# blackccpie/another_raytracer

Hardware: AMD Instinct MI355X
Metric: Msamples/sec (primary+secondary rays) at 1920x1080x1024spp; 1/2/4/8 GPU (higher is better)
Workload: dtype f64

## Files before the change

### another_raytracer_amd/_lib.py

```python
import ctypes
import os

try:
    import torch
except ImportError:
    pass

_HERE = os.path.dirname(os.path.abspath(__file__))
LIB_PATH = os.environ.get("ART_LIB") or os.path.join(_HERE, "libart.so")

RT_OK = 0
RT_FP64 = 0
RT_ABI_VERSION = 5
RT_OUT_DEVICE, RT_PROFILE, RT_GLOBAL_SCENE, RT_SPLIT_SHADE, RT_ADAPTIVE, RT_WAVEFRONT, RT_PARALLEL_IMAGES = 1, 2, 4, 8, 16, 32, 64
RT_GUIDE_DOUBLES = 10
RT_DN_NO_DEMODULATE = 256
RT_Q_ANY_HIT, RT_Q_NO_MEDIA = 512, 1024
RT_HIT_DOUBLES = 12
ERRORS = {-1: "RT_E_INVALID", -2: "RT_E_SCENE", -3: "RT_E_DEVICE", -4: "RT_E_INTERNAL"}


class rt_camera(ctypes.Structure):
    _fields_ = [("lookfrom", ctypes.c_double * 3), ("lookat", ctypes.c_double * 3), ("vup", ctypes.c_double * 3),
                ("vfov", ctypes.c_double), ("aspect", ctypes.c_double), ("aperture", ctypes.c_double),
# ... 77 lines not shown
    "rt_option_set": (_I, [ctypes.c_char_p, _D]),
    "rt_option_get": (_I, [ctypes.c_char_p, _DP]),
    "rt_scene_build": (_I, [ctypes.c_char_p, ctypes.c_char_p, _I, ctypes.POINTER(_P)]),
    "rt_scene_info_get": (_I, [_P, ctypes.POINTER(rt_scene_info)]),
    "rt_scene_dump": (_S, [_P, ctypes.c_char_p, _S]),
    "rt_scene_destroy": (None, [_P]),
    "rt_scene_save": (_I, [_P, ctypes.c_char_p]),
    "rt_scene_load": (_I, [ctypes.c_char_p, _I, ctypes.POINTER(_P)]),
    "rt_render": (_I, [_P, ctypes.POINTER(rt_camera), ctypes.POINTER(rt_params), _P, _P, ctypes.POINTER(rt_stats)]),
    "rt_render_progressive": (_I, [_P, ctypes.POINTER(rt_camera), ctypes.POINTER(rt_params), _P, _P, rt_progress_fn, _P,
                                   ctypes.POINTER(rt_stats)]),
    "rt_trace_rays": (_I, [_P, _P, ctypes.c_int64, ctypes.c_int32, _P, _P]),
    "rt_query_rays": (_I, [_P, ctypes.POINTER(rt_query_params), _P, _P, ctypes.c_int64, _P, _P]),
    "rt_radiance_rays": (_I, [_P, ctypes.POINTER(rt_radiance_params), _P, _P, ctypes.c_int64, _P, ctypes.POINTER(rt_stats)]),
    "rt_camera_rays": (_I, [ctypes.POINTER(rt_camera), ctypes.POINTER(rt_params), ctypes.c_uint32, _I, _P, _P]),
    "rt_render_views": (_I, [_P, ctypes.POINTER(rt_camera), _P, ctypes.c_int32, ctypes.POINTER(rt_params), _P, _P, ctypes.POINTER(rt_stats)]),
    "rt_render_guides": (_I, [_P, ctypes.POINTER(rt_camera), ctypes.POINTER(rt_params), _P, _P]),
    "rt_denoise": (_I, [_I, ctypes.POINTER(rt_denoise_params), _P, _P, ctypes.c_int32, _P, _P, _P, _DP]),
    "rt_render_denoised": (_I, [_P, ctypes.POINTER(rt_camera), ctypes.POINTER(rt_params), ctypes.POINTER(rt_denoise_params), _P, _P,
                                ctypes.POINTER(rt_stats)]),
    "rt_render_noise_target": (_I, [_P, ctypes.POINTER(rt_camera), ctypes.POINTER(rt_params), ctypes.POINTER(rt_noise_params), _P, _P, _P, _P,
                                    ctypes.POINTER(rt_stats), ctypes.POINTER(rt_noise_result)]),
    "rt_image_load": (_I, [ctypes.c_char_p, ctypes.POINTER(ctypes.c_int32), ctypes.POINTER(ctypes.c_int32), ctypes.POINTER(ctypes.c_int32),
                           ctypes.POINTER(ctypes.POINTER(ctypes.c_uint8))]),
    "rt_image_free": (None, [ctypes.POINTER(ctypes.c_uint8)]),
    "rt_local_rows": (_I, [ctypes.POINTER(rt_params), ctypes.POINTER(ctypes.c_int32)]),
    "rt_band_block_rows": (_I, [ctypes.c_int32, ctypes.c_int32, ctypes.c_int32]),
    "rt_unpack_bands": (_I, [_P, _S, _P, _S, ctypes.c_int32, ctypes.c_int32, ctypes.c_int32, ctypes.c_int32, ctypes.c_int32, _P]),
    "rt_multi_create": (_I, [ctypes.c_char_p, ctypes.c_char_p, _IP, _I, ctypes.POINTER(_P)]),
    "rt_multi_from_graph": (_I, [_P, _IP, _I, ctypes.POINTER(_P)]),
# ... 133 lines not shown
```

### another_raytracer_amd/csrc/abi.cpp

```cpp
#include <chrono>
#include <cmath>
#include <cstdlib>
#include <cstring>
#include <exception>
#include <stdexcept>
#include <memory>
#include <new>
#include <string>
#include <vector>

#include "art.h"
#include "denoise.h"
#include "imagedec.h"
#include "multi.h"
#include "renderer.h"
#include "scenefile.h"
#include "objmesh.h"
#include "options.h"
#include "pass_plan.h"
#include "scene.h"

namespace art {
int device_count();
}
// ... 373 lines not shown
    if (view_paths > art::kMaxPassSlots)
        return fail(RT_E_INVALID, "rt_render_views: one view of width * height * spp = " + std::to_string(view_paths) + " paths exceeds kMaxPassSlots = "
                                  "2^31 paths per launch: render such frames with rt_render, which splits a frame into passes");
    if (nviews == 0) return RT_OK;
    if (!out_rgb8) return fail(RT_E_INVALID, "rt_render_views: out_rgb8 must be non-NULL");
    return guard(RT_E_DEVICE, [&] {
        std::vector<art::CameraRec> recs(static_cast<size_t>(nviews));
        for (int32_t v = 0; v < nviews; ++v) recs[static_cast<size_t>(v)] = camera_of(&cams[v]);
        art::RenderStats st;
        s->device_renderer().render_views(recs.data(), seeds, static_cast<size_t>(nviews), render_params(p), out_rgb8, out_accum, stats ? &st : nullptr);
        if (stats) {
            fill_stats(st, stats);
            stats->extend_variant = stats->kernel_lds_mode = -1;
        }
        return RT_OK;
    });
}

int rt_camera_rays(const rt_camera* cam, const rt_params* p, uint32_t sample_base, int device, double* rays_out, uint64_t* rng_out) {
    std::string why;
    if (!cam || !rays_out) return fail(RT_E_INVALID, "rt_camera_rays: camera and rays_out must be non-NULL");
    if (!p) return fail(RT_E_INVALID, "params is NULL");
    if (device < 0) return fail(RT_E_INVALID, "device must be >= 0");
    rt_params q = *p;
    q.max_depth = 0;
    if (!valid_params(&q, why)) return fail(RT_E_INVALID, why);
    if (p->flags & ~RT_OUT_DEVICE) return fail(RT_E_INVALID, "rt_camera_rays takes RT_OUT_DEVICE only");
    if (p->stream && !(p->flags & RT_OUT_DEVICE)) return fail(RT_E_INVALID, "rt_camera_rays: stream needs RT_OUT_DEVICE");
    const uint64_t rows = static_cast<uint64_t>(art::band_local_rows(p->height, p->band_rows, p->band_count, p->band_index));
    const uint64_t npix_pad = static_cast<uint64_t>((p->width + 7) / 8) * ((rows + 7) / 8) * 64u;
// ... 365 lines not shown
```

### another_raytracer_amd/csrc/device_scene.h

```cpp
#pragma once
#include <algorithm>
#include <vector>

#include "hip_check.h"
#include "path_work.h"
#include "scene.h"

namespace art {

struct DeviceScene {
    std::vector<void*> allocs;
    DevScene view{};
    bool media = false;
    uint32_t features = F_ALL;
    int max_stack = kMaxStackDepth;
    uint32_t mat_types = (1u << kNumMatTypes) - 1;
    bool tex_basic = false;
    bool lds_scene = false;
    bool lds_shade = false;
    bool codes16 = false;
    uint32_t leaf_shift = 0;
    bool tex_bary = false;
    size_t bytes = 0;

    template <class T>
    const T* upload(const std::vector<T>& v) {
        if (v.empty()) return nullptr;
        void* p = nullptr;
        HIP_OK(hipMalloc(&p, v.size() * sizeof(T)));
        HIP_OK(hipMemcpy(p, v.data(), v.size() * sizeof(T), hipMemcpyHostToDevice));
        allocs.push_back(p);
        bytes += v.size() * sizeof(T);
        return static_cast<const T*>(p);
    }
// ... 15 lines not shown
```

### another_raytracer_amd/csrc/device_scene.hip

```cpp
#include "device_scene.h"

#include <cmath>
#include <cstring>
#include <limits>
#include <unordered_map>

#include "options.h"

namespace art {

static std::vector<uint8_t> lds_scene_image(const FlatScene& f, uint32_t& nmov, bool& shade_ok) {
    std::vector<uint8_t> img;
    nmov = 0;
    shade_ok = false;
    if ((f.features & ~kFeatSpheres) != 0 || f.nodes.empty() || f.nodes.size() > kLdsNodeCap || f.primrefs.size() > kLdsSlotCap ||
        f.world.size() > kPathsWorldCap || f.objs.size() > kPathsWorldCap ||
        f.spheres.size() > kLdsRefIndexMask || std::max(extend_lds_bytes(true, stack_rows(f.max_stack)), paths_lds_bytes(stack_rows(f.max_stack))) > kLdsPerCu)
        return img;
    for (int32_t w : f.world)
        if (w < 0 || static_cast<size_t>(w) >= f.objs.size() || f.objs[w].kind != OBJ_BVH) return img;
    for (uint32_t ref : f.primrefs) {
        if (primref_type(ref) != PRIM_SPHERE) return img;
        const SphereRec& sp = f.spheres[primref_index(ref)];
        if (sp.flags & SPH_MOVING) {
            if (sp.t0 != 0.0 || sp.dt != 1.0 || sp.d[0] != 0.0 || sp.d[2] != 0.0) return img;
            ++nmov;
        }
    }
// ... 65 lines not shown
            } else if (mat.type == MAT_DIELECTRIC) {
                const double inv = 1.0 / mat.ir;
                double r0f = (1.0 - inv) / (1.0 + inv), r0b = (1.0 - mat.ir) / (1.0 + mat.ir);
                r0f = r0f * r0f;
                r0b = r0b * r0b;
                const double d3[3] = {inv, r0f, r0b};
                entry[sp.mat] = static_cast<int32_t>(put_entry(d3, mat.ir));
            } else {
                shade_ok = false;
            }
        }
        const uint16_t mi = static_cast<uint16_t>(entry[sp.mat] < 0 ? 0 : entry[sp.mat]);
        put(kLdsOffMatIdx + sl * 2, &mi, 2);
    }
    if (nent > kLdsMatCap) shade_ok = false;
    return img;
}


static std::vector<uint32_t> pair_align_leaves(const std::vector<uint32_t>& primrefs, std::vector<BvhNode>& nodes,
                                               std::vector<ObjRec>& objs, std::vector<uint8_t>& pad) {
    std::vector<std::pair<uint32_t, uint32_t>> leaves;
    for (const BvhNode& b : nodes)
        for (int c = 0; c < 4; ++c)
            if (b.child[c] < 0 && b.child[c] != kNodeEmpty) leaves.emplace_back(leaf_first(b.child[c]), leaf_count(b.child[c]));
    for (const auto& o : objs)
        if (o.kind == OBJ_BVH && o.b != kNodeEmpty) leaves.emplace_back(leaf_first(o.b), leaf_count(o.b));
    std::sort(leaves.begin(), leaves.end());
    leaves.erase(std::unique(leaves.begin(), leaves.end()), leaves.end());
    std::unordered_map<uint32_t, uint32_t> moved;
// ... 161 lines not shown
    }
    ds.view.world = ds.upload(f.world);
    ds.view.mats = ds.upload(mats);
    ds.view.texs = ds.upload(f.texs);
    ds.view.perlins = ds.upload(f.perlins);
    {
        std::vector<uint8_t> ib(kUvTableBytes + sizeof(ImageRec) * f.images.size(), 0);
        std::memcpy(ib.data(), glibc_trig_data::kTrigHost, sizeof(glibc_trig_data::kTrigHost));
        if (!f.images.empty()) std::memcpy(ib.data() + kUvTableBytes, f.images.data(), sizeof(ImageRec) * f.images.size());
        ds.view.images = reinterpret_cast<const ImageRec*>(ds.upload(ib) + kUvTableBytes);
    }
    ds.view.texels = ds.upload(f.texels);
    {
        uint32_t nmov = 0;
        bool shade_ok = false;
        const std::vector<uint8_t> img = ds.leaf_shift ? std::vector<uint8_t>() : lds_scene_image(f, nmov, shade_ok);
        if (!img.empty()) {
            ds.view.lds_image = ds.upload(img);
            ds.lds_scene = true;
            ds.lds_shade = shade_ok;
        }
    }
    ds.view.n_nodes = static_cast<uint32_t>(f.nodes.size());
    ds.view.n_objs = static_cast<uint32_t>(f.objs.size());
    ds.view.n_mats = static_cast<uint32_t>(f.mats.size());
    ds.view.n_primrefs = static_cast<uint32_t>(f.primrefs.size());
    ds.view.n_tris = static_cast<uint32_t>(f.tris.size());
    ds.view.nworld = static_cast<int32_t>(f.world.size());
    for (int a = 0; a < 3; ++a) ds.view.bg[a] = f.background[a];
    ds.media = f.has_media;
    ds.features = f.features;
// ... 25 lines not shown
```

### another_raytracer_amd/csrc/k_paths.hip

```cpp
#include "launch.h"
#include "path_pool.h"
#include "path_work.h"

namespace art {

struct __align__(16) PoolRay {
    double2 a, b, c;
    double2 d, e;
    uint64_t rng;
    uint32_t slot, depth;
};
static_assert(sizeof(PoolRay) == 96, "pool entries are six 16-B pieces");
struct PathPool {
    PoolRay* base;
    uint32_t count;
    uint32_t cur, end;
    bool exhausted;
    __device__ __forceinline__ void init(void* pool, uint32_t block, uint32_t nblocks, uint32_t waves_per_block, uint32_t w) {
        const uint32_t per_xcd = (nblocks + kXcds - 1) / kXcds;
        const uint32_t wave = ((block % kXcds) * per_xcd + block / kXcds) * waves_per_block + w;
        base = static_cast<PoolRay*>(pool) + static_cast<size_t>(wave) * kPoolCap;
        count = cur = end = 0;
        exhausted = false;
    }
    __device__ __forceinline__ bool batch(const PassGeom& sg, const CameraRec& sc, uint32_t* next_slot, uint32_t lane, PathState& st,
                                          uint32_t& q) {
        if (cur == end) {
            const uint32_t chunk = sg.chunk;
            uint32_t nb = 0;
            if (lane == 0) nb = atomicAdd(next_slot, chunk);
            nb = __builtin_amdgcn_readfirstlane(nb);
            cur = nb;
            end = nb + chunk;
        }
        const uint32_t b = cur;
        cur += 64;
        q = b + lane;
        __asm__ volatile("" ::: "memory");
        if (b + 64u >= sg.P) exhausted = true;
        int lx, ly;
        uint32_t qi, j;
        slot_split(sg, q, qi, j);
        if (!(q < sg.P && slot_pixel(sg, qi, lx, ly))) return false;
        cam_ray(sg, sc, j, lx, ly, st.ray, st.rng);
        st.T = mk(1.0, 1.0, 1.0);
        return true;
    }
    __device__ __forceinline__ void push(uint64_t m, uint32_t rank, bool busy, const PathState& st, uint32_t q, int depth) {
        if (busy) {
            PoolRay& e = base[pool_push_pos(count, rank)];
            e.a = make_double2(st.ray.o.x, st.ray.o.y);
            e.b = make_double2(st.ray.o.z, st.ray.d.x);
            e.c = make_double2(st.ray.d.y, st.ray.d.z);
            e.d = make_double2(st.ray.tm, st.T.x);
            e.e = make_double2(st.T.y, st.T.z);
            e.rng = st.rng;
            e.slot = q;
// ... 2 lines not shown
        count += static_cast<uint32_t>(__popcll(m));
        __asm__ volatile("" ::: "memory");
    }
    __device__ __forceinline__ void pop(uint32_t rank, PathState& st, uint32_t& q, int& depth) const {
        const PoolRay& e = base[pool_pop_pos(count, rank)];
        const double2 a = e.a, b = e.b, c = e.c, d = e.d, f = e.e;
        st.ray.o = mk(a.x, a.y, b.x);
        st.ray.d = mk(b.y, c.x, c.y);
        st.ray.tm = d.x;
        st.T = mk(d.y, f.x, f.y);
        st.rng = e.rng;
        q = e.slot;
        depth = static_cast<int>(e.depth);
    }
};
__global__ __launch_bounds__(kBlockL, 1) void k_paths(DevScene S0, PassGeom g, CameraRec cam, Work w, uint32_t* next_slot) {
    constexpr int B = kBlockL;
    extern __shared__ __align__(16) uint8_t smem[];
    const uint8_t* lds = smem;
    StackT<true>* stk = reinterpret_cast<StackT<true>*>(smem + kLdsImageBytes) + B + stack_column<true>(threadIdx.x);
    JumpEntry* jt = reinterpret_cast<JumpEntry*>(smem + kLdsImageBytes + paths_stack_bytes(g.stack));
    CameraRec& s_cam = *reinterpret_cast<CameraRec*>(smem + kLdsImageBytes + paths_stack_bytes(g.stack) + kJumpBytes);
    PassGeom& s_g = *reinterpret_cast<PassGeom*>(smem + kLdsImageBytes + paths_stack_bytes(g.stack) + kJumpBytes + sizeof(CameraRec));
    stk[-B] = static_cast<StackT<true>>(kNodeEmpty);
    load_lds_image<B>(S0.lds_image, smem);
    if (threadIdx.x < static_cast<uint32_t>(kJumpEntries)) jt[threadIdx.x] = pcg_jump(3u * threadIdx.x);
    if (threadIdx.x == 0) {
        s_cam = cam;
        s_g = g;
        if (g.list_mode) {
// ... 12 lines not shown
        S.world = reinterpret_cast<const int32_t*>(wb);
        S.objs = reinterpret_cast<const ObjRec*>(ob);
    }
    __syncthreads();
    const uint32_t lane = __lane_id();
    const uint64_t below = (1ull << lane) - 1ull;
    const V3 bg = mk(S.bg[0], S.bg[1], S.bg[2]);
    bool busy = false;
    uint32_t q = 0;
    int depth = 0;
    PathState st;
    unsigned long long segs = 0;
#ifdef ART_STATS
    unsigned long long tm_load = 0, tm_trace = 0, tm_shade = 0, tm_app = 0, tm_fb = 0, tm_prev = __builtin_amdgcn_s_memtime();
#endif
    PathPool pp;
    pp.init(w.pool, blockIdx.x, gridDim.x, B / 64, threadIdx.x / 64);
    for (;;) {
        const uint64_t m_busy = __ballot(busy);
        const uint32_t n_idle = 64u - static_cast<uint32_t>(__popcll(m_busy));
        const bool fb = pool_batch_due(pp.exhausted, pp.count, n_idle);
        bool act;
        if (fb) {
#ifdef ART_STATS
            if (lane == 0) atomicAdd(&g_art_stats[51], static_cast<unsigned long long>(__popcll(m_busy)));
#endif
            if (m_busy) pp.push(m_busy, static_cast<uint32_t>(__popcll(m_busy & below)), busy, st, q, depth);
            act = pp.batch(s_g, s_cam, next_slot, lane, st, q);
            depth = 0;
        } else {
            const uint32_t npop = pool_pop_count(pp.count, n_idle);
            if (npop) {
                const uint32_t rank = static_cast<uint32_t>(__popcll(~m_busy & below));
                if (!busy && rank < npop) {
                    pp.pop(rank, st, q, depth);
                    busy = true;
                }
                pp.count -= npop;
            } else if (m_busy == 0) {
                ART_TICK(tm_load);
                break;
            }
            act = busy;
        }
        ART_TICK((fb ? tm_fb : tm_load));
        double t = 0.0;
        HitOut h{0, 0, kMatUnknown};
        bool hitw = false;
        if (act) {
            ++segs;
            hitw = trace_world<kFeatSpheres, B, true>(S, lds, st.ray, stk, st.rng, t, h);
#if ART_LDS_LEAF_NOREF
            if (hitw) h.mt = reinterpret_cast<const uint32_t*>(lds + kLdsOffRef)[h.obj >> 16] >> kLdsRefMatShift;
#endif
        }
        __asm__ volatile("s_waitcnt vmcnt(0)" ::: "memory");
        ART_TICK((fb ? tm_fb : tm_trace));
        const bool need = act && hitw && (h.mt == MAT_LAMBERTIAN || h.mt == MAT_METAL) && depth + 1 < g.max_depth;
        const V3 ps = coop_unit_sphere(need, st.rng, jt);
        bool cont = false;
        if (act) {
            st.L = mk(0.0, 0.0, 0.0);
            if (hitw) {
                cont = shade_hit_lds(lds, h.obj >> 16, h.mt, t, depth + 1 >= g.max_depth, st, &ps);
            } else {
                st.L = st.L + st.T * bg;
// ... 46 lines not shown
```

### another_raytracer_amd/csrc/kernels_unity.hip

```cpp
#include "kernels.hip"
#include "k_paths.hip"
#include "k_paths_g_mesh.hip"
#include "radiance_rays.hip"
#include "device_scene.hip"
#include "renderer.hip"
```

### another_raytracer_amd/csrc/launch.h

```cpp
#pragma once
#include <functional>

#include "device_scene.h"
#include "path_work.h"

namespace art {

enum ExtendVariant { EXT_GLOBAL = 0, EXT_LDS = 1, EXT_FUSED = 2, EXT_MEGA = 3, EXT_MEGA_G = 4 };
int extend_variant(const DeviceScene& ds, int flags);
struct KernelId {
    uint32_t f = 0, tf = 0;
    int lm = -1;
};

bool static_lds_is_zero(const void* kernel);
int blocks_per_cu(const void* kernel, int block, size_t lds);
KernelId launch_paths_g(uint32_t feat, bool tex_basic, bool tex_bary, bool codes16, uint32_t leaf_shift, int num_cu, hipStream_t st,
                        const DevScene& S, const PassGeom& g, const CameraRec& cam, const Work& w, uint32_t* next_slot);
void bounce(const DeviceScene& ds, int variant, int num_cu, hipStream_t st, const PassGeom& g, const CameraRec& cam,
            const Work& w, int d, const std::function<void()>& mark);
void launch_accum(hipStream_t st, const PassGeom& g, const Work& w, double* qsum, uint32_t m);
void launch_finalize(hipStream_t st, const double* acc, uint8_t* rgb, uint32_t n, int spp);
void launch_adapt_corners(hipStream_t st, uint32_t* list, int W, int sqx, uint32_t nsq);
void launch_adapt_store(hipStream_t st, const uint32_t* list, uint32_t n, const double* acc, int spp, int32_t* work);
// ... 33 lines not shown
    ResRec* res;
    uint32_t* next;
    unsigned long long* segments;
    uint32_t P, spp, chunk;
    uint32_t npix;
    uint32_t stack;
    int32_t max_depth;
    int32_t W, H;
    double inv_w1, inv_h1;
    FastDiv fd_spp, fd_npix, fd_w;
};
void launch_radiance_views(const DeviceScene& ds, int flags, int num_cu, hipStream_t st, const ViewsJob& job, uint32_t npixels, const double background[3]);
void launch_camera_rays(hipStream_t st, const PassGeom& g, const CameraRec& cam, double* rays, uint64_t* rng);
void launch_paths(int num_cu, hipStream_t st, const DevScene& S, const PassGeom& g, const CameraRec& cam, const Work& w,
                  uint32_t* next_slot);
size_t pool_bytes(int variant, int num_cu);

}
```

### another_raytracer_amd/csrc/options.cpp

```cpp
#include "options.h"

#include <algorithm>
#include <atomic>
#include <cmath>
#include <cstdlib>
#include <cstring>
#include <limits>

namespace art {

namespace {

struct OptDef {
    const char* name;
    double def, lo, hi;
    bool integer;
};
constexpr double kInf = std::numeric_limits<double>::infinity();
const OptDef kDefs[static_cast<int>(Opt::kCount)] = {
    {"compile.world_merge", 2, 0, 2, true},
    {"compile.hoist", 1, 0, 1, true},
    {"bvh.collapse", 0, 0, 1, true},
    {"bvh.collapse_ci", 0.6, 0, 1e6, false},
    {"bvh.dp_binary_leaf", 1, 1, 16, true},
    {"bvh.sah_ci", 1.5, 0, 1e6, false},
    {"bvh.sah_leaf", 4, 1, 16, true},
    {"bvh.sbvh", 1.5, 0, 1e6, false},
    {"bvh.sbvh_alpha", 1e-5, 0, 1e6, false},
    {"render.codes16", 1, 0, 1, true},
    {"render.lds_nodes_max", 4294967295.0, 0, 4294967295.0, true},
    {"render.leaf2", 1, 0, 1, true},
    {"render.tex_bary", 1, 0, 1, true},
    {"denoise.lds_iterations", 2, 0, 2, true},
    {"query.any_sorted", 0, 0, 1, true},
    {"views.max_paths", 0, 0, 2147483648.0, true},
    {"multi.timeout_ms", std::numeric_limits<double>::quiet_NaN(), 0, kInf, false},
    {"multi.rccl_blocking", 0, 0, 1, true},
    {"test.fault_workspace_bytes", 0, 0, 1.8e19, true},
    {"test.fault_gather_abort", 0, 0, 1, true},
    {"test.fault_rccl_group", 0, 0, 2, true},
};

std::atomic<double> g_val[static_cast<int>(Opt::kCount)];
std::atomic<bool> g_init{false};

void init_once() {
    if (g_init.load(std::memory_order_acquire)) return;
    static const bool done = [] {
        opt_reset_all();
        g_init.store(true, std::memory_order_release);
// ... 54 lines not shown
```

### another_raytracer_amd/csrc/options.h

```cpp
#pragma once
#include <cstddef>

namespace art {

enum class Opt : int {
    WorldMerge,
    Hoist,
    BvhCollapse,
    CollapseCi,
    DpBinaryLeaf,
    SahCi,
    SahLeaf,
    Sbvh,
    SbvhAlpha,
    Codes16,
    LdsNodesMax,
    Leaf2,
    TexBary,
    DenoiseLdsIterations,
    QueryAnySorted,
    ViewsMaxPaths,
    MultiTimeoutMs,
    RcclBlocking,
    FaultWorkspaceBytes,
    FaultGatherAbort,
    FaultRcclGroup,
    kCount
};

double opt(Opt o);
bool opt_set(const char* name, double value, const char** why);
bool opt_get(const char* name, double* value);
void opt_reset_all();

}
```

### another_raytracer_amd/csrc/path_work.h

```cpp
#pragma once
#include <hip/hip_runtime.h>

#include <cstdint>

#include "device.h"
#include "pass_plan.h"

namespace art {

struct PathRec {
    double2 a, b, c, e;
    double2 f, g, h, i;
};
static_assert(sizeof(PathRec) == 128, "PathRec is two 64-B lines");
struct PathState {
    Ray ray;
    V3 T, L;
    uint64_t rng;
};
__device__ __forceinline__ void load_path(const PathRec* P, uint32_t q, PathState& s, bool full) {
    const PathRec& p = P[q];
    const double2 a = p.a, b = p.b, c = p.c, e = p.e;
    s.ray.o = mk(a.x, a.y, b.x);
    s.ray.d = mk(b.y, c.x, c.y);
// ... 79 lines not shown
    uint32_t nlist;
    uint32_t chunk;
    uint32_t lds_ring;
    uint32_t list_mode;
};
struct Work {
    PathRec* paths;
    HitRecD* hits;
    ResRec* res;
    uint32_t* active[2];
    uint32_t* mq;
    uint32_t* counters;
    unsigned long long* segments;
    double* acc;
    void* pool;
};
__host__ __device__ __forceinline__ uint32_t* counter(const Work& w, int d, int kind, int s) {
    return w.counters + (static_cast<size_t>((d * kQueueKinds + kind) * kShards + s)) * kCounterStride;
}

__device__ __forceinline__ int global_row(const PassGeom& g, int ly) {
    const uint32_t b = g.fd_band_rows.div(static_cast<uint32_t>(ly));
    return static_cast<int>(b) * (g.band_rows * g.band_count) + g.band_index * g.band_rows + (ly - static_cast<int>(b) * g.band_rows);
}
__device__ __forceinline__ void slot_split(const PassGeom& g, uint32_t slot, uint32_t& qi, uint32_t& j) {
    const uint32_t a = g.fd_npix.div(slot), b = slot - a * g.npix_pad;
    qi = g.list_mode ? a : b;
    j = g.list_mode ? b : a;
}
__device__ __forceinline__ bool slot_pixel(const PassGeom& g, uint32_t qi, int& lx, int& ly) {
// ... 268 lines not shown
```

### another_raytracer_amd/csrc/renderer.h

```cpp
#pragma once
#include <cstdint>
#include <functional>

#include "art.h"
#include "layout.h"
#include "noise_target.h"
#include "scene.h"

namespace art {

struct RenderParams {
    int width = 0, height = 0, spp = 1, max_depth = 50;
    uint64_t seed = 0;
    int fp_mode = RT_FP64;
    int band_rows = 1, band_count = 1, band_index = 0;
    int samples_per_pass = 0;
    int flags = 0;
    void* stream = nullptr;
    double background[3] = {0, 0, 0};
    std::function<bool(int samples_done)> on_pass;
};

struct RenderStats {
    uint64_t segments = 0, primary = 0;
// ... 21 lines not shown
    ~Renderer();
    Renderer(const Renderer&) = delete;
    Renderer& operator=(const Renderer&) = delete;
    void upload();
    void render(const CameraRec& cam, const RenderParams& p, uint8_t* out_rgb, double* out_acc, RenderStats& stats);
    void trace_rays(const double* rays, size_t n, bool global_scene, double* t_out, double* n_out);
    void query_rays(const double* rays, const double* t_max, size_t n, bool device, bool global_scene, bool any_hit, bool no_media, void* stream,
                    double* hits, uint8_t* occluded);
    void radiance_rays(const RadianceParams& p, const double* rays, const uint64_t* rng, size_t n, double* radiance, RenderStats* stats);
    void render_views(const CameraRec* cams, const uint64_t* seeds, size_t nviews, const RenderParams& p, uint8_t* out_rgb, double* out_acc,
                      RenderStats* stats);
    static void camera_rays(int device, const CameraRec& cam, const RenderParams& p, uint32_t sample_base, double* rays_out, uint64_t* rng_out);
    void render_guides(const CameraRec& cam, const RenderParams& p, double* guides, double* rays_out);
    void render_noise_target(const CameraRec& cam, const RenderParams& p, const NoiseParams& np, uint8_t* out_rgb, double* out_acc,
                             int32_t* out_count, double* out_moments, RenderStats& stats, NoiseResult& result);
    int device() const;
    size_t scene_bytes() const;
    const FlatScene& flat() const;

private:
    Impl* impl_;
};

}
```

### another_raytracer_amd/csrc/renderer.hip

```cpp
#include "renderer.h"

#include <algorithm>
#include <cstdio>
#include <cstdlib>
#include <cstring>
#include <vector>

#include "launch.h"
#include "options.h"
#include "pass_plan.h"
#include "view_plan.h"
#include "workspace.h"

namespace art {

struct Renderer::Impl {
    int device = 0;
    int num_cu = 256;
    hipStream_t own_stream = nullptr;
    FlatScene flat;
    DeviceScene s64;
    bool up64 = false;
    DeviceBuffer ws{true};
    hipEvent_t ev[2] = {nullptr, nullptr};
    std::vector<ViewRec> view_table;
// ... 35 lines not shown
    g.band_index = p.band_index;
    g.tiles_x = static_cast<uint32_t>((p.width + 7) / 8);
    const uint32_t tiles_y = static_cast<uint32_t>((nrows + 7) / 8);
    g.npix_pad = g.tiles_x * tiles_y * 64u;
    g.max_depth = p.max_depth;
    g.seed = p.seed;
    g.seed_mix = splitmix64(p.seed);
    g.fd_tiles_x = FastDiv::make(g.tiles_x);
    g.fd_band_rows = FastDiv::make(static_cast<uint32_t>(p.band_rows));
    g.fd_w = FastDiv::make(static_cast<uint32_t>(p.width));
    g.fd_npix = FastDiv::make(g.npix_pad);
    g.inv_w1 = 1.0 / static_cast<double>(p.width - 1);
    g.inv_h1 = 1.0 / static_cast<double>(p.height - 1);
    g.stack = stack;
    return g;
}
static size_t counter_words(int max_depth) { return static_cast<size_t>(std::max(max_depth + 1, 4)) * kQueueKinds * kShards * kCounterStride; }

struct ProfileMarks {
    std::vector<hipEvent_t> ev;
    size_t used = 0;
    ~ProfileMarks() { for (auto e : ev) if (e) (void)hipEventDestroy(e); }
    void reserve(size_t n) {
        while (ev.size() < n) {
            ev.push_back(nullptr);
            HIP_OK(hipEventCreate(&ev.back()));
        }
    }
    void mark(hipStream_t stream) {
        reserve(used + 1);
// ... 258 lines not shown
    launch_adapt_fill(f.stream, b.ad_work, f.drgb, p.width, f.nrows, b.sqx, b.ad_f0, b.ad_f1, b.ad_f2);
    return traced * static_cast<uint64_t>(b.spp_t);
}

void Renderer::render(const CameraRec& cam, const RenderParams& p, uint8_t* out_rgb, double* out_acc, RenderStats& stats) {
    if (p.fp_mode != RT_FP64) throw std::runtime_error("fp_mode must be RT_FP64");
    upload();
    Impl& I = *impl_;
    Frame f{I, I.s64, cam, p};
    const bool images = (p.flags & RT_PARALLEL_IMAGES) != 0, adaptive = (p.flags & RT_ADAPTIVE) != 0;
    RenderBufs b{};
    b.spp_t = images ? 4 * (p.spp / 4) : p.spp, b.out_rgb = out_rgb, b.out_acc = out_acc;
#ifdef ART_TRACE
    trace_setup();
#endif
    if (!begin_frame(f, stats, b.spp_t, true, adaptive ? 4 : 1, [&](Carver& c) {
        const bool wf = !f.mega;
        f.w.paths = c.take<PathRec>(f.Pmax, wf);
        f.w.hits = c.take<HitRecD>(f.Pmax, wf);
        f.w.res = c.take<ResRec>(f.Pmax);
        f.w.active[0] = c.take<uint32_t>(static_cast<size_t>(kShards) * f.g.cap, wf);
        f.w.active[1] = c.take<uint32_t>(static_cast<size_t>(kShards) * f.g.cap, wf);
        f.w.mq = c.take<uint32_t>(static_cast<size_t>(kMatSegs) * f.g.cap, wf);
        f.w.counters = c.take<uint32_t>(counter_words(p.max_depth));
        f.w.segments = c.take<unsigned long long>(1);
        f.w.acc = c.take<double>(3 * f.local_pix);
        f.drgb = c.take<uint8_t>(3 * f.local_pix);
        double* qsum = c.take<double>(3 * f.local_pix, images);
        b.qsum = images ? qsum : nullptr;
        f.w.pool = c.take<char>(pool_bytes(f.variant, I.num_cu));
        b.ad_work = c.take<int32_t>(3 * f.local_pix, adaptive);
        b.ad_lists = c.take<uint32_t>(f.local_pix + 4 * 64, adaptive);
        b.ad_f0 = c.take<uint8_t>(21 * (f.local_pix / (kBig * kBig)), adaptive);
        b.ad_count = c.take<uint32_t>(1, adaptive);
    })) return;
    b.ad_f1 = b.ad_f0 + f.local_pix / (kBig * kBig), b.ad_f2 = b.ad_f1 + 4 * (f.local_pix / (kBig * kBig));
    b.sqx = p.width / kBig, b.nsq = static_cast<uint32_t>(b.sqx) * static_cast<uint32_t>(f.nrows / kBig);
    uint32_t ad_counts[4] = {0, 0, 0, 0};
    uint64_t primary = 0;
    if (!adaptive) primary = render_whole(f, b);
    else if (f.mega && f.k == static_cast<uint32_t>(b.spp_t) && !images && !p.on_pass) adaptive_device_counted(f, b, ad_counts);
    else primary = adaptive_host_counted(f, b);
    end_frame(f, stats, out_rgb, adaptive ? nullptr : out_acc);
    stats.primary = primary + (static_cast<uint64_t>(ad_counts[0]) + ad_counts[1] + ad_counts[2] + ad_counts[3]) * static_cast<uint64_t>(b.spp_t);
}

void Renderer::upload() {
    HIP_OK(hipSetDevice(impl_->device));
    if (!impl_->up64) {
        build_device_scene(impl_->flat, impl_->s64);
        impl_->up64 = true;
    }
}

void Renderer::trace_rays(const double* rays, size_t n, bool global_scene, double* t_out, double* n_out) {
    upload();
    const DeviceScene& ds = impl_->s64;
    if (n == 0) return;
    if (n > (1u << 30)) throw std::runtime_error("too many rays");
// ... 330 lines not shown
```

### another_raytracer_amd/engine.py

```python
import ctypes
import enum

import numpy as np

from ._lib import RT_ADAPTIVE, RT_DN_NO_DEMODULATE, RT_FP64, RT_GUIDE_DOUBLES, rt_denoise_params, RT_PARALLEL_IMAGES, rt_progress_fn, RT_GLOBAL_SCENE, RT_OUT_DEVICE, RT_PROFILE, RT_SPLIT_SHADE, RT_WAVEFRONT, check, dvec, lib, rt_camera, rt_params, rt_stats
from .scene import compile_world


class tracer_constants:
    aspect_ratio = 4.0 / 3.0
    image_width = 720
    image_height = int(image_width / aspect_ratio)
    color_channels = 3
    samples_per_pixel = 100
    max_depth = 50


class engine_mode(enum.Enum):
    single = 0
    adaptive = 1
    parallel_stripes = 2
    parallel_images = 3


# ... 135 lines not shown
        rows = check(lib.rt_local_rows(ctypes.byref(p), None), "rt_local_rows")
        nbytes = rows * self.width * 3
        ptr, dev = _pointer(output_image, nbytes)
        acc_ptr = None
        if accum is not None:
            acc_ptr, acc_dev = _pointer(accum.view(np.uint8) if isinstance(accum, np.ndarray) else accum, nbytes * 8)
            if acc_dev != dev:
                raise ValueError("output_image and accum must both live on the host or both on the device")
        if dev:
            p.flags |= RT_OUT_DEVICE
        st = rt_stats()
        check(lib.rt_render(self._scene, ctypes.byref(self.cam.c), ctypes.byref(p), ctypes.c_void_p(ptr),
                            ctypes.c_void_p(acc_ptr) if acc_ptr else None, ctypes.byref(st)), "engine.run")
        self.stats = st.as_dict()
        return int(round(st.ms))

    def render_guides(self, guides=None, rays=None, band_rows=None, band_count=1, band_index=0, stream=None):
        if self._scene is None:
            raise ValueError("no scene set")
        p = self.params(band_rows, band_count, band_index, RT_GLOBAL_SCENE if self.global_scene else 0, stream)
        rows = check(lib.rt_local_rows(ctypes.byref(p), None), "rt_local_rows")
        n = rows * self.width
        if guides is None:
            guides = np.empty((rows, self.width, RT_GUIDE_DOUBLES), np.float64)
        ptr, dev = _f64_pointer(guides, RT_GUIDE_DOUBLES * n, "guides")
        rays_ptr = None
        if rays is not None:
            rays_ptr, rays_dev = _f64_pointer(rays, 7 * n, "rays")
            if rays_dev != dev:
                raise ValueError("guides and rays must both live on the host or both on the device")
# ... 126 lines not shown
```

### include/art.h

```cpp
#ifndef ART_H
#define ART_H

#include <stddef.h>
#include <stdint.h>

#ifdef __cplusplus
extern "C" {
#endif

#define RT_ABI_VERSION 5

#define RT_OK 0
#define RT_E_INVALID (-1)
#define RT_E_SCENE (-2)
#define RT_E_DEVICE (-3)
#define RT_E_INTERNAL (-4)

#define RT_FP64 0
#define RT_OUT_DEVICE 1
#define RT_PROFILE 2
#define RT_GLOBAL_SCENE 4
#define RT_SPLIT_SHADE 8
#define RT_ADAPTIVE 16
#define RT_WAVEFRONT 32
// ... 79 lines not shown
int rt_query_rays(rt_scene* scene, const rt_query_params* q, const double* rays, const double* t_max, int64_t n, double* hits,
                  uint8_t* occluded);
typedef struct rt_radiance_params {
    int32_t flags;
    int32_t spp;
    int32_t max_depth;
    uint32_t sample_base;
    uint64_t seed;
    uint64_t id_base;
    void* stream;
    double background[3];
} rt_radiance_params;
int rt_radiance_rays(rt_scene* scene, const rt_radiance_params* q, const double* rays, const uint64_t* rng, int64_t n, double* radiance,
                     rt_stats* stats);
int rt_camera_rays(const rt_camera* cam, const rt_params* params, uint32_t sample_base, int device, double* rays_out, uint64_t* rng_out);
int rt_render_views(rt_scene* scene, const rt_camera* cams, const uint64_t* seeds, int32_t nviews, const rt_params* params, uint8_t* out_rgb8,
                    double* out_accum, rt_stats* stats);
int rt_local_rows(const rt_params* params, int32_t* rows_out);
int rt_band_block_rows(int32_t height, int32_t band_rows, int32_t n);
int rt_unpack_bands(const uint8_t* packed, size_t packed_bytes, uint8_t* frame, size_t frame_bytes, int32_t width, int32_t height,
                    int32_t band_rows, int32_t n, int32_t flags, void* stream);

#define RT_GUIDE_DOUBLES 10
int rt_render_guides(rt_scene* scene, const rt_camera* cam, const rt_params* params, double* guides, double* rays_out);
#define RT_DN_NO_DEMODULATE 256
typedef struct rt_denoise_params {
    int32_t width, height;
    int32_t iterations;
    int32_t normal_squarings;
    double sigma_color;
// ... 84 lines not shown
```

Baseline: 20430.

## Cull primary rays per 8x8 tile with precomputed sphere candidate lists

Adds a pre-pass kernel that builds, for each 8x8 pixel tile, a depth-sorted list of up to 15 spheres whose conservative cone bound, padded for lens and motion blur, can reach the tile. In the megakernel, first-bounce rays intersect only that short list from LDS instead of walking the full BVH, and tiles that overflow fall back to the normal traversal. It is on by default for LDS-resident sphere scenes at 72 spp or more, and adds an extra launch plus a debug API. Correctness depends on the conservative bound staying valid.

```diff
diff --git a/another_raytracer_amd/_lib.py b/another_raytracer_amd/_lib.py
--- a/another_raytracer_amd/_lib.py
+++ b/another_raytracer_amd/_lib.py
@@ -115,6 +115,7 @@
     "rt_query_rays": (_I, [_P, ctypes.POINTER(rt_query_params), _P, _P, ctypes.c_int64, _P, _P]),
     "rt_radiance_rays": (_I, [_P, ctypes.POINTER(rt_radiance_params), _P, _P, ctypes.c_int64, _P, ctypes.POINTER(rt_stats)]),
     "rt_camera_rays": (_I, [ctypes.POINTER(rt_camera), ctypes.POINTER(rt_params), ctypes.c_uint32, _I, _P, _P]),
+    "rt_tile_candidates": (_I, [_P, ctypes.POINTER(rt_camera), ctypes.POINTER(rt_params), _P, ctypes.c_int64]),
     "rt_render_views": (_I, [_P, ctypes.POINTER(rt_camera), _P, ctypes.c_int32, ctypes.POINTER(rt_params), _P, _P, ctypes.POINTER(rt_stats)]),
     "rt_render_guides": (_I, [_P, ctypes.POINTER(rt_camera), ctypes.POINTER(rt_params), _P, _P]),
     "rt_denoise": (_I, [_I, ctypes.POINTER(rt_denoise_params), _P, _P, ctypes.c_int32, _P, _P, _P, _DP]),
diff --git a/another_raytracer_amd/csrc/abi.cpp b/another_raytracer_amd/csrc/abi.cpp
--- a/another_raytracer_amd/csrc/abi.cpp
+++ b/another_raytracer_amd/csrc/abi.cpp
@@ -411,6 +411,22 @@
             stats->extend_variant = stats->kernel_lds_mode = -1;
         }
         return RT_OK;
+    });
+}
+
+int rt_tile_candidates(rt_scene* s, const rt_camera* cam, const rt_params* p, uint16_t* counts_out, int64_t cap) {
+    std::string why;
+    if (!s || !cam) return fail(RT_E_INVALID, "rt_tile_candidates: scene and camera must be non-NULL");
+    if (!valid_params(p, why)) return fail(RT_E_INVALID, why);
+    if (counts_out && cap < 0) return fail(RT_E_INVALID, "rt_tile_candidates: cap must be >= 0");
+    if (counts_out) {
+        const int64_t rows = art::band_local_rows(p->height, p->band_rows, p->band_count, p->band_index);
+        const int64_t tiles = static_cast<int64_t>((p->width + 7) / 8) * ((rows + 7) / 8);
+        if (cap < tiles) return fail(RT_E_INVALID, "rt_tile_candidates: counts_out holds " + std::to_string(cap) + " entries, the frame has " +
+                                                       std::to_string(tiles) + " tiles");
+    }
+    return guard(RT_E_DEVICE, [&] {
+        return s->device_renderer().tile_candidates(camera_of(cam), render_params(p), counts_out, static_cast<size_t>(counts_out ? cap : 0));
     });
 }
 
diff --git a/another_raytracer_amd/csrc/device_scene.h b/another_raytracer_amd/csrc/device_scene.h
--- a/another_raytracer_amd/csrc/device_scene.h
+++ b/another_raytracer_amd/csrc/device_scene.h
@@ -18,6 +18,7 @@
     bool tex_basic = false;
     bool lds_scene = false;
     bool lds_shade = false;
+    uint32_t tile_reps = 0;
     bool codes16 = false;
     uint32_t leaf_shift = 0;
     bool tex_bary = false;
diff --git a/another_raytracer_amd/csrc/device_scene.hip b/another_raytracer_amd/csrc/device_scene.hip
--- a/another_raytracer_amd/csrc/device_scene.hip
+++ b/another_raytracer_amd/csrc/device_scene.hip
@@ -6,12 +6,14 @@
 #include <unordered_map>
 
 #include "options.h"
+#include "tile_lists.h"
 
 namespace art {
 
-static std::vector<uint8_t> lds_scene_image(const FlatScene& f, uint32_t& nmov, bool& shade_ok) {
+static std::vector<uint8_t> lds_scene_image(const FlatScene& f, uint32_t& nmov, bool& shade_ok, uint32_t& tile_reps) {
     std::vector<uint8_t> img;
     nmov = 0;
+    tile_reps = 0;
     shade_ok = false;
     if ((f.features & ~kFeatSpheres) != 0 || f.nodes.empty() || f.nodes.size() > kLdsNodeCap || f.primrefs.size() > kLdsSlotCap ||
         f.world.size() > kPathsWorldCap || f.objs.size() > kPathsWorldCap ||
@@ -107,6 +109,28 @@
         put(kLdsOffMatIdx + sl * 2, &mi, 2);
     }
     if (nent > kLdsMatCap) shade_ok = false;
+    TileReps reps{};
+    {
+        std::unordered_map<uint32_t, uint32_t> first;
+        bool same = shade_ok;
+        auto eq = [&](uint32_t off, uint32_t stride, uint32_t a, uint32_t b) { return std::memcmp(img.data() + off + a * stride, img.data() + off + b * stride, stride) == 0; };
+        for (uint32_t sl = 0; sl < f.primrefs.size(); ++sl) {
+            const uint32_t idx = primref_index(f.primrefs[sl]);
+            const auto it = first.find(idx);
+            if (it == first.end()) {
+                first.emplace(idx, sl);
+                reps.slot[reps.n++] = static_cast<uint16_t>(sl);
+                continue;
+            }
+            const uint32_t r = it->second;
+            same = same && eq(kLdsOffSph, 16, sl, r) && eq(kLdsOffSph + kLdsSlotCap * 16, 16, sl, r) && eq(kLdsOffMov, 8, sl, r) &&
+                   eq(kLdsOffRef, 4, sl, r) && eq(kLdsOffMatIdx, 2, sl, r) && eq(kLdsOffInvR, 8, sl, r);
+        }
+        if (!same) reps.n = 0;
+    }
+    img.resize(kLdsImageBytes + sizeof(TileReps));
+    std::memcpy(img.data() + kLdsImageBytes, &reps, sizeof reps);
+    tile_reps = reps.n;
     return img;
 }
 
@@ -298,7 +322,9 @@
     {
         uint32_t nmov = 0;
         bool shade_ok = false;
-        const std::vector<uint8_t> img = ds.leaf_shift ? std::vector<uint8_t>() : lds_scene_image(f, nmov, shade_ok);
+        uint32_t tile_reps = 0;
+        const std::vector<uint8_t> img = ds.leaf_shift ? std::vector<uint8_t>() : lds_scene_image(f, nmov, shade_ok, tile_reps);
+        ds.tile_reps = img.empty() ? 0 : tile_reps;
         if (!img.empty()) {
             ds.view.lds_image = ds.upload(img);
             ds.lds_scene = true;
diff --git a/another_raytracer_amd/csrc/k_paths.hip b/another_raytracer_amd/csrc/k_paths.hip
--- a/another_raytracer_amd/csrc/k_paths.hip
+++ b/another_raytracer_amd/csrc/k_paths.hip
@@ -1,6 +1,7 @@
 #include "launch.h"
 #include "path_pool.h"
 #include "path_work.h"
+#include "tile_lists.h"
 
 namespace art {
 
@@ -24,7 +25,7 @@
         exhausted = false;
     }
     __device__ __forceinline__ bool batch(const PassGeom& sg, const CameraRec& sc, uint32_t* next_slot, uint32_t lane, PathState& st,
-                                          uint32_t& q) {
+                                          uint32_t& q, uint32_t& tile) {
         if (cur == end) {
             const uint32_t chunk = sg.chunk;
             uint32_t nb = 0;
@@ -41,6 +42,7 @@
         int lx, ly;
         uint32_t qi, j;
         slot_split(sg, q, qi, j);
+        tile = __builtin_amdgcn_readfirstlane(qi >> 6);
         if (!(q < sg.P && slot_pixel(sg, qi, lx, ly))) return false;
         cam_ray(sg, sc, j, lx, ly, st.ray, st.rng);
         st.T = mk(1.0, 1.0, 1.0);
@@ -73,6 +75,31 @@
         depth = static_cast<int>(e.depth);
     }
 };
+typedef uint32_t u32x8 __attribute__((ext_vector_type(8)));
+__device__ __forceinline__ bool trace_tile_list(const uint8_t* lds, const Ray& r, u32x8 rec, double& t, HitOut& h) {
+    const double d_a = len2(r.d), d_inv_a = 1.0 / d_a;
+    uint64_t q0 = rec[0] | (static_cast<uint64_t>(rec[1]) << 32), q1 = rec[2] | (static_cast<uint64_t>(rec[3]) << 32);
+    uint64_t q2 = rec[4] | (static_cast<uint64_t>(rec[5]) << 32), q3 = rec[6] | (static_cast<uint64_t>(rec[7]) << 32);
+    const uint32_t n = static_cast<uint32_t>(q0) & 0xFFFFu;
+    double closest = __builtin_inf();
+    bool any = false;
+    for (uint32_t k = 0; k < n; ++k) {
+        q0 = (q0 >> 16) | (q1 << 48), q1 = (q1 >> 16) | (q2 << 48), q2 = (q2 >> 16) | (q3 << 48), q3 >>= 16;
+        const uint32_t slot = static_cast<uint32_t>(q0) & 0xFFFFu;
+        double tt;
+        uint32_t prim, mt;
+        if (hit_lds_slot(lds, slot, r, d_a, d_inv_a, 0.001, closest, tt, prim, mt)) {
+            closest = tt;
+            any = true;
+            h.prim = prim;
+            h.obj = slot << 16;
+            h.mt = mt;
+        }
+    }
+    t = closest;
+    return any;
+}
+
 __global__ __launch_bounds__(kBlockL, 1) void k_paths(DevScene S0, PassGeom g, CameraRec cam, Work w, uint32_t* next_slot) {
     constexpr int B = kBlockL;
     extern __shared__ __align__(16) uint8_t smem[];
@@ -115,6 +142,8 @@
 #ifdef ART_STATS
     unsigned long long tm_load = 0, tm_trace = 0, tm_shade = 0, tm_app = 0, tm_fb = 0, tm_prev = __builtin_amdgcn_s_memtime();
 #endif
+    const bool lists = w.tiles != nullptr && g.list == nullptr;
+    uint32_t tile = 0;
     PathPool pp;
     pp.init(w.pool, blockIdx.x, gridDim.x, B / 64, threadIdx.x / 64);
     for (;;) {
@@ -127,7 +156,7 @@
             if (lane == 0) atomicAdd(&g_art_stats[51], static_cast<unsigned long long>(__popcll(m_busy)));
 #endif
             if (m_busy) pp.push(m_busy, static_cast<uint32_t>(__popcll(m_busy & below)), busy, st, q, depth);
-            act = pp.batch(s_g, s_cam, next_slot, lane, st, q);
+            act = pp.batch(s_g, s_cam, next_slot, lane, st, q, tile);
             depth = 0;
         } else {
             const uint32_t npop = pool_pop_count(pp.count, n_idle);
@@ -150,7 +179,12 @@
         bool hitw = false;
         if (act) {
             ++segs;
-            hitw = trace_world<kFeatSpheres, B, true>(S, lds, st.ray, stk, st.rng, t, h);
+            u32x8 rec = {kTileOverflow, 0, 0, 0, 0, 0, 0, 0};
+            if (fb && lists)
+                rec = *(reinterpret_cast<const __attribute__((address_space(4))) u32x8*>(reinterpret_cast<uintptr_t>(w.tiles)) +
+                        __builtin_amdgcn_readfirstlane(tile));
+            if ((rec[0] & 0xFFFFu) != kTileOverflow) hitw = trace_tile_list(lds, st.ray, rec, t, h);
+            else hitw = trace_world<kFeatSpheres, B, true>(S, lds, st.ray, stk, st.rng, t, h);
 #if ART_LDS_LEAF_NOREF
             if (hitw) h.mt = reinterpret_cast<const uint32_t*>(lds + kLdsOffRef)[h.obj >> 16] >> kLdsRefMatShift;
 #endif
diff --git a/another_raytracer_amd/csrc/kernels_unity.hip b/another_raytracer_amd/csrc/kernels_unity.hip
--- a/another_raytracer_amd/csrc/kernels_unity.hip
+++ b/another_raytracer_amd/csrc/kernels_unity.hip
@@ -2,5 +2,6 @@
 #include "k_paths.hip"
 #include "k_paths_g_mesh.hip"
 #include "radiance_rays.hip"
+#include "tile_lists.hip"
 #include "device_scene.hip"
 #include "renderer.hip"
diff --git a/another_raytracer_amd/csrc/launch.h b/another_raytracer_amd/csrc/launch.h
--- a/another_raytracer_amd/csrc/launch.h
+++ b/another_raytracer_amd/csrc/launch.h
@@ -71,6 +71,7 @@
 void launch_camera_rays(hipStream_t st, const PassGeom& g, const CameraRec& cam, double* rays, uint64_t* rng);
 void launch_paths(int num_cu, hipStream_t st, const DevScene& S, const PassGeom& g, const CameraRec& cam, const Work& w,
                   uint32_t* next_slot);
+void launch_tile_lists(hipStream_t st, const DevScene& S, const PassGeom& g, const CameraRec& cam, void* tiles);
 size_t pool_bytes(int variant, int num_cu);
 
 }
diff --git a/another_raytracer_amd/csrc/options.cpp b/another_raytracer_amd/csrc/options.cpp
--- a/another_raytracer_amd/csrc/options.cpp
+++ b/another_raytracer_amd/csrc/options.cpp
@@ -34,6 +34,7 @@
     {"denoise.lds_iterations", 2, 0, 2, true},
     {"query.any_sorted", 0, 0, 1, true},
     {"views.max_paths", 0, 0, 2147483648.0, true},
+    {"render.tile_lists", 1, 0, 2, true},
     {"multi.timeout_ms", std::numeric_limits<double>::quiet_NaN(), 0, kInf, false},
     {"multi.rccl_blocking", 0, 0, 1, true},
     {"test.fault_workspace_bytes", 0, 0, 1.8e19, true},
diff --git a/another_raytracer_amd/csrc/options.h b/another_raytracer_amd/csrc/options.h
--- a/another_raytracer_amd/csrc/options.h
+++ b/another_raytracer_amd/csrc/options.h
@@ -20,6 +20,7 @@
     DenoiseLdsIterations,
     QueryAnySorted,
     ViewsMaxPaths,
+    TileLists,
     MultiTimeoutMs,
     RcclBlocking,
     FaultWorkspaceBytes,
diff --git a/another_raytracer_amd/csrc/path_work.h b/another_raytracer_amd/csrc/path_work.h
--- a/another_raytracer_amd/csrc/path_work.h
+++ b/another_raytracer_amd/csrc/path_work.h
@@ -117,6 +117,7 @@
     unsigned long long* segments;
     double* acc;
     void* pool;
+    const void* tiles;
 };
 __host__ __device__ __forceinline__ uint32_t* counter(const Work& w, int d, int kind, int s) {
     return w.counters + (static_cast<size_t>((d * kQueueKinds + kind) * kShards + s)) * kCounterStride;
diff --git a/another_raytracer_amd/csrc/renderer.h b/another_raytracer_amd/csrc/renderer.h
--- a/another_raytracer_amd/csrc/renderer.h
+++ b/another_raytracer_amd/csrc/renderer.h
@@ -59,6 +59,7 @@
     void render_guides(const CameraRec& cam, const RenderParams& p, double* guides, double* rays_out);
     void render_noise_target(const CameraRec& cam, const RenderParams& p, const NoiseParams& np, uint8_t* out_rgb, double* out_acc,
                              int32_t* out_count, double* out_moments, RenderStats& stats, NoiseResult& result);
+    int tile_candidates(const CameraRec& cam, const RenderParams& p, uint16_t* counts, size_t cap);
     int device() const;
     size_t scene_bytes() const;
     const FlatScene& flat() const;
diff --git a/another_raytracer_amd/csrc/renderer.hip b/another_raytracer_amd/csrc/renderer.hip
--- a/another_raytracer_amd/csrc/renderer.hip
+++ b/another_raytracer_amd/csrc/renderer.hip
@@ -9,6 +9,7 @@
 #include "launch.h"
 #include "options.h"
 #include "pass_plan.h"
+#include "tile_lists.h"
 #include "view_plan.h"
 #include "workspace.h"
 
@@ -74,6 +75,11 @@
     g.inv_h1 = 1.0 / static_cast<double>(p.height - 1);
     g.stack = stack;
     return g;
+}
+constexpr uint32_t kTileListsAutoSpp = 72;
+static bool tile_lists_wanted(const DeviceScene& ds, int variant, uint32_t k) {
+    const int mode = static_cast<int>(opt(Opt::TileLists));
+    return variant == EXT_MEGA && ds.tile_reps > 0 && (mode == 2 || (mode == 1 && k >= kTileListsAutoSpp));
 }
 static size_t counter_words(int max_depth) { return static_cast<size_t>(std::max(max_depth + 1, 4)) * kQueueKinds * kShards * kCounterStride; }
 
@@ -362,6 +368,7 @@
 #ifdef ART_TRACE
     trace_setup();
 #endif
+    TileRec* tile_tab = nullptr;
     if (!begin_frame(f, stats, b.spp_t, true, adaptive ? 4 : 1, [&](Carver& c) {
         const bool wf = !f.mega;
         f.w.paths = c.take<PathRec>(f.Pmax, wf);
@@ -377,6 +384,7 @@
         double* qsum = c.take<double>(3 * f.local_pix, images);
         b.qsum = images ? qsum : nullptr;
         f.w.pool = c.take<char>(pool_bytes(f.variant, I.num_cu));
+        tile_tab = c.take<TileRec>(f.g.npix_pad / 64u, !adaptive && tile_lists_wanted(f.ds, f.variant, f.k));
         b.ad_work = c.take<int32_t>(3 * f.local_pix, adaptive);
         b.ad_lists = c.take<uint32_t>(f.local_pix + 4 * 64, adaptive);
         b.ad_f0 = c.take<uint8_t>(21 * (f.local_pix / (kBig * kBig)), adaptive);
@@ -386,11 +394,43 @@
     b.sqx = p.width / kBig, b.nsq = static_cast<uint32_t>(b.sqx) * static_cast<uint32_t>(f.nrows / kBig);
     uint32_t ad_counts[4] = {0, 0, 0, 0};
     uint64_t primary = 0;
+    if (!adaptive && p.max_depth > 0 && tile_lists_wanted(f.ds, f.variant, f.k)) {
+        launch_tile_lists(f.stream, f.ds.view, f.g, cam, tile_tab);
+        f.w.tiles = tile_tab;
+    }
     if (!adaptive) primary = render_whole(f, b);
     else if (f.mega && f.k == static_cast<uint32_t>(b.spp_t) && !images && !p.on_pass) adaptive_device_counted(f, b, ad_counts);
     else primary = adaptive_host_counted(f, b);
     end_frame(f, stats, out_rgb, adaptive ? nullptr : out_acc);
     stats.primary = primary + (static_cast<uint64_t>(ad_counts[0]) + ad_counts[1] + ad_counts[2] + ad_counts[3]) * static_cast<uint64_t>(b.spp_t);
+}
+
+int Renderer::tile_candidates(const CameraRec& cam, const RenderParams& p, uint16_t* counts, size_t cap) {
+    upload();
+    Impl& I = *impl_;
+    DeviceScene& ds = I.s64;
+    const int nrows = band_local_rows(p.height, p.band_rows, p.band_count, p.band_index);
+    if (nrows == 0 || p.max_depth <= 0 || (p.flags & RT_ADAPTIVE)) return 0;
+    const PassGeom g = make_pass_geom(p, nrows, stack_rows(ds.max_stack));
+    if (g.npix_pad > kMaxPassSlots) throw std::runtime_error("image too large for one pass (more than 2^31 padded pixels)");
+    const int variant = extend_variant(ds, p.flags);
+    size_t free_b = 0, total_b = 0;
+    HIP_OK(hipMemGetInfo(&free_b, &total_b));
+    const int spp_t = (p.flags & RT_PARALLEL_IMAGES) ? 4 * (p.spp / 4) : p.spp;
+    const PassPlan plan = plan_passes((free_b + I.ws.size()) / 2 / sizeof(ResRec), p.samples_per_pass, g.npix_pad, spp_t, true);
+    if (!tile_lists_wanted(ds, variant, plan.k)) return 0;
+    const size_t ntiles = g.npix_pad / 64u;
+    if (!counts) return static_cast<int>(ntiles);
+    if (cap < ntiles) throw std::runtime_error("rt_tile_candidates: counts holds fewer entries than the frame has tiles");
+    Carver c(I.ws.reserve(sizeof(TileRec) * ntiles));
+    TileRec* tab = c.take<TileRec>(ntiles);
+    launch_tile_lists(I.own_stream, ds.view, g, cam, tab);
+    HIP_OK(hipGetLastError());
+    std::vector<TileRec> host(ntiles);
+    HIP_OK(hipMemcpyAsync(host.data(), tab, sizeof(TileRec) * ntiles, hipMemcpyDeviceToHost, I.own_stream));
+    HIP_OK(hipStreamSynchronize(I.own_stream));
+    for (size_t i = 0; i < ntiles; ++i) counts[i] = host[i].n;
+    return static_cast<int>(ntiles);
 }
 
 void Renderer::upload() {
diff --git a/another_raytracer_amd/csrc/tile_lists.h b/another_raytracer_amd/csrc/tile_lists.h
--- /dev/null
+++ b/another_raytracer_amd/csrc/tile_lists.h
@@ -0,0 +1,91 @@
+#pragma once
+#include <cmath>
+#include <cstdint>
+
+#include "layout.h"
+
+namespace art {
+
+constexpr uint32_t kTileK = 15;
+constexpr uint16_t kTileOverflow = 0xFFFF;
+constexpr double kTilePad = 1e-6, kTileFar = 1e8;
+struct alignas(32) TileRec {
+    uint16_t n;
+    uint16_t slot[kTileK];
+};
+static_assert(sizeof(TileRec) == 32, "a tile record is 32 B");
+struct TileReps {
+    uint32_t n;
+    uint16_t slot[kLdsSlotCap];
+    uint16_t pad[6];
+};
+static_assert(sizeof(TileReps) % 16 == 0, "uploaded behind the 16-B aligned image");
+
+struct TileFrame {
+    int32_t W, H, band_rows, band_count, band_index;
+    uint32_t tiles_x;
+};
+struct TileBundle {
+    double O[3], D[3];
+    double DD;
+    double r_lens, r_tile;
+    double t_mid, t_half;
+};
+
+ART_HD TileBundle tile_bundle(const CameraRec& cam, const TileFrame& g, uint32_t tile) {
+    const uint32_t ty = tile / g.tiles_x, tx = tile - ty * g.tiles_x;
+    const double s0 = static_cast<double>(8 * tx) / static_cast<double>(g.W - 1), s1 = static_cast<double>(8 * tx + 8) / static_cast<double>(g.W - 1);
+    const int gmin = band_global_row(static_cast<int>(8 * ty), g.band_rows, g.band_count, g.band_index);
+    const int gmax = band_global_row(static_cast<int>(8 * ty + 7), g.band_rows, g.band_count, g.band_index);
+    const double t0 = static_cast<double>(g.H - 1 - gmax) / static_cast<double>(g.H - 1), t1 = static_cast<double>(g.H - gmin) / static_cast<double>(g.H - 1);
+    const double sc = 0.5 * (s0 + s1), tc = 0.5 * (t0 + t1), sh = 0.5 * (s1 - s0), th = 0.5 * (t1 - t0);
+    TileBundle b;
+    double hh = 0, vv = 0, uu = 0, ww = 0, uw = 0;
+    b.DD = 0;
+    for (int a = 0; a < 3; ++a) {
+        b.O[a] = cam.origin[a];
+        b.D[a] = cam.llc[a] + sc * cam.horizontal[a] + tc * cam.vertical[a] - cam.origin[a];
+        b.DD += b.D[a] * b.D[a];
+        hh += cam.horizontal[a] * cam.horizontal[a];
+        vv += cam.vertical[a] * cam.vertical[a];
+        uu += cam.u[a] * cam.u[a];
+        ww += cam.v[a] * cam.v[a];
+        uw += cam.u[a] * cam.v[a];
+    }
+    b.r_tile = sh * std::sqrt(hh) + th * std::sqrt(vv);
+    b.r_lens = std::fabs(cam.lens_radius) * std::sqrt((uu > ww ? uu : ww) + std::fabs(uw));
+    b.t_mid = 0.5 * (cam.time0 + cam.time1);
+    b.t_half = 0.5 * std::fabs(cam.time1 - cam.time0);
+    return b;
+}
+
+ART_HD bool tile_piece(double ww, double wD, double DD, double k0, double k1, double lo, double hi, double& first) {
+    const double a = DD - k1 * k1, hb = wD - k0 * k1, c = ww - k0 * k0;
+    first = lo;
+    if ((a * lo + 2.0 * hb) * lo + c <= 0.0) return true;
+    if (hi >= 0.0 && (a * hi + 2.0 * hb) * hi + c <= 0.0) return true;
+    if (!(a > 0.0)) return hi < 0.0;
+    const double tv = -hb / a;
+    if (!(tv > lo) || (hi >= 0.0 && !(tv < hi))) return false;
+    const double disc = hb * hb - a * c;
+    if (disc < 0.0) return false;
+    first = (-hb - std::sqrt(disc)) / a;
+    if (!(first > lo)) first = lo;
+    return true;
+}
+
+ART_HD bool tile_reaches(const TileBundle& b, double cx, double cy, double cz, double r, double dy, double& key) {
+    const double my = cy + b.t_mid * dy, rad = std::fabs(r) + b.t_half * std::fabs(dy);
+    const double w[3] = {b.O[0] - cx, b.O[1] - my, b.O[2] - cz};
+    const double ww = w[0] * w[0] + w[1] * w[1] + w[2] * w[2], wD = w[0] * b.D[0] + w[1] * b.D[1] + w[2] * b.D[2];
+    key = 0.0;
+    if (!(ww < kTileFar * kTileFar * rad * rad)) return true;
+    const double R = rad + kTilePad * (rad + std::sqrt(ww) + std::sqrt(b.DD));
+    double f0, f1;
+    const bool p0 = tile_piece(ww, wD, b.DD, R + b.r_lens, b.r_tile - b.r_lens, 0.0, 1.0, f0);
+    const bool p1 = tile_piece(ww, wD, b.DD, R - b.r_lens, b.r_tile + b.r_lens, 1.0, -1.0, f1);
+    key = p0 ? f0 : f1;
+    return p0 || p1;
+}
+
+}
diff --git a/another_raytracer_amd/csrc/tile_lists.hip b/another_raytracer_amd/csrc/tile_lists.hip
--- /dev/null
+++ b/another_raytracer_amd/csrc/tile_lists.hip
@@ -0,0 +1,67 @@
+#include "launch.h"
+#include "tile_lists.h"
+
+namespace art {
+
+constexpr int kTileBlock = 256, kTileWaves = kTileBlock / 64;
+
+__global__ __launch_bounds__(kTileBlock) void k_tile_lists(const uint8_t* image, CameraRec cam, TileFrame g, uint32_t ntiles, TileRec* out) {
+    __shared__ double s_key[kTileWaves][kTileK + 1];
+    __shared__ uint16_t s_slot[kTileWaves][kTileK + 1];
+    __shared__ uint16_t s_out[kTileWaves][kTileK + 1];
+    const uint32_t wv = threadIdx.x >> 6, lane = threadIdx.x & 63u;
+    const uint32_t tile_w = blockIdx.x * kTileWaves + wv;
+    const bool live = tile_w < ntiles;
+    const uint32_t tile = live ? tile_w : 0u;
+    const TileReps* reps = reinterpret_cast<const TileReps*>(image + kLdsImageBytes);
+    const uint32_t n = reps->n <= kLdsSlotCap ? reps->n : 0u;
+    const TileBundle b = tile_bundle(cam, g, tile);
+    const uint64_t below = (1ull << lane) - 1ull;
+    if (lane <= kTileK) s_out[wv][lane] = 0;
+    uint32_t count = 0;
+    for (uint32_t i0 = 0; i0 < n; i0 += 64) {
+        const uint32_t i = i0 + lane;
+        bool cand = false;
+        double key = 0.0;
+        uint32_t slot = 0;
+        if (i < n) {
+            slot = reps->slot[i] & (kLdsSlotCap - 1);
+            const double2 a = reinterpret_cast<const double2*>(image + kLdsOffSph)[slot];
+            const double2 c = reinterpret_cast<const double2*>(image + kLdsOffSph)[kLdsSlotCap + slot];
+            const double dy = reinterpret_cast<const double*>(image + kLdsOffMov)[slot];
+            cand = tile_reaches(b, a.x, a.y, c.x, sqrt(c.y), dy, key);
+        }
+        const uint64_t m = __ballot(cand);
+        const uint32_t rank = count + static_cast<uint32_t>(__popcll(m & below));
+        if (cand && rank <= kTileK) {
+            s_key[wv][rank] = key;
+            s_slot[wv][rank] = static_cast<uint16_t>(slot);
+        }
+        count += static_cast<uint32_t>(__popcll(m));
+    }
+    __syncthreads();
+    const bool over = count > kTileK;
+    if (!over && lane < count) {
+        const double key = s_key[wv][lane];
+        uint32_t rank = 0;
+        for (uint32_t j = 0; j < count; ++j) {
+            const double kj = s_key[wv][j];
+            rank += (kj < key || (kj == key && j < lane)) ? 1u : 0u;
+        }
+        s_out[wv][1u + rank] = s_slot[wv][lane];
+    }
+    __syncthreads();
+    if (live && lane <= kTileK) {
+        uint16_t* rec = reinterpret_cast<uint16_t*>(out + tile);
+        rec[lane] = lane == 0 ? (over ? kTileOverflow : static_cast<uint16_t>(count)) : (over ? uint16_t(0) : s_out[wv][lane]);
+    }
+}
+
+void launch_tile_lists(hipStream_t st, const DevScene& S, const PassGeom& g, const CameraRec& cam, void* tiles) {
+    const uint32_t ntiles = g.npix_pad / 64u;
+    const TileFrame tf{g.W, g.H, g.band_rows, g.band_count, g.band_index, g.tiles_x};
+    hipLaunchKernelGGL(k_tile_lists, dim3((ntiles + kTileWaves - 1) / kTileWaves), dim3(kTileBlock), 0, st, S.lds_image, cam, tf, ntiles,
+                       static_cast<TileRec*>(tiles));
+}
+
+}
diff --git a/another_raytracer_amd/engine.py b/another_raytracer_amd/engine.py
--- a/another_raytracer_amd/engine.py
+++ b/another_raytracer_amd/engine.py
@@ -173,6 +173,20 @@
                             ctypes.c_void_p(acc_ptr) if acc_ptr else None, ctypes.byref(st)), "engine.run")
         self.stats = st.as_dict()
         return int(round(st.ms))
+
+    def tile_candidates(self, band_rows=None, band_count=1, band_index=0):
+        if self._scene is None:
+            raise ValueError("no scene set")
+        flags = ((RT_GLOBAL_SCENE if self.global_scene else 0) | (RT_SPLIT_SHADE if self.split_shade else 0)
+                 | (RT_ADAPTIVE if self.m == engine_mode.adaptive else 0)
+                 | (RT_PARALLEL_IMAGES if self.m == engine_mode.parallel_images else 0) | (RT_WAVEFRONT if self.wavefront else 0))
+        p = self.params(band_rows, band_count, band_index, flags)
+        rows = check(lib.rt_local_rows(ctypes.byref(p), None), "rt_local_rows")
+        tx, ty = (self.width + 7) // 8, (rows + 7) // 8
+        counts = np.zeros((ty, tx), np.uint16)
+        n = check(lib.rt_tile_candidates(self._scene, ctypes.byref(self.cam.c), ctypes.byref(p), ctypes.c_void_p(counts.ctypes.data), tx * ty),
+                  "engine.tile_candidates")
+        return counts if n else None
 
     def render_guides(self, guides=None, rays=None, band_rows=None, band_count=1, band_index=0, stream=None):
         if self._scene is None:
diff --git a/include/art.h b/include/art.h
--- a/include/art.h
+++ b/include/art.h
@@ -117,6 +117,7 @@
 int rt_radiance_rays(rt_scene* scene, const rt_radiance_params* q, const double* rays, const uint64_t* rng, int64_t n, double* radiance,
                      rt_stats* stats);
 int rt_camera_rays(const rt_camera* cam, const rt_params* params, uint32_t sample_base, int device, double* rays_out, uint64_t* rng_out);
+int rt_tile_candidates(rt_scene* scene, const rt_camera* cam, const rt_params* params, uint16_t* counts_out, int64_t cap);
 int rt_render_views(rt_scene* scene, const rt_camera* cams, const uint64_t* seeds, int32_t nviews, const rt_params* params, uint8_t* out_rgb8,
                     double* out_accum, rt_stats* stats);
 int rt_local_rows(const rt_params* params, int32_t* rows_out);
```

Result: faster. 23340, median of 6 (+14.2%).
